# MarkTakken/kf2vecFSW

Hardware: AMD Instinct MI355X
Metric: Gbases/s k-mer→.kf build at k=7; achieved HBM GB/s vs gfx950 peak (higher is better)
Workload: dtype u32

## Files before the change

kf2vecfsw_amd/build.py:

```python
from __future__ import annotations

import hashlib
import os
import subprocess
import sys

HERE = os.path.dirname(os.path.abspath(__file__))
CSRC = os.path.join(HERE, "csrc")
OUT = os.path.join(HERE, "libkf2vec_gpu.so")
BUILD = os.path.join(HERE, "_build")
ARCH = os.environ.get("KF_OFFLOAD_ARCH", "gfx950")
HIPCC = os.environ.get("HIPCC", "/opt/rocm/bin/hipcc")

SOURCES_HIP = ["kf_count.hip", "kf_bucket.hip", "kf_chunks.hip", "kf_sparse.hip", "kf_index.hip", "kf_rows.hip",
               "kf_kmers.hip", "kf_merge.hip", "kf_chunkfeat.hip", "kf_kfparse.hip"]
SOURCES_CPP = ["kf_host.cpp"]
DEPS = SOURCES_HIP + SOURCES_CPP + ["kf_internal.h", "kf_front.h", "kf_scan.h", "kf_compact.h", "../../include/kf2vec_gpu.h"]


def source_id() -> str:
    h = hashlib.sha256(ARCH.encode())
    for d in sorted(DEPS):
        h.update(b"\0" + os.path.basename(d).encode() + b"\0")
        with open(os.path.join(CSRC, d), "rb") as f:
            h.update(f.read())
    return h.hexdigest()[:16]


def embedded_id(path: str) -> str | None:
    try:
        with open(path, "rb") as f:
            blob = f.read()
    except OSError:
        return None
    i = blob.find(b"KF_BUILD_ID=")
    if i < 0:
        return None
    j = blob.find(b"\0", i)
    return blob[i + 12: j].decode(errors="replace")


def _stale() -> bool:
    return embedded_id(OUT) != source_id()


def build(force: bool = False, verbose: bool = False, ablation: bool = False, out: str | None = None) -> str:
    import fcntl
    out = out or OUT
    if not force and not ablation and out == OUT and not _stale():
        return OUT
    os.makedirs(BUILD, exist_ok=True)
    with open(os.path.join(BUILD, ".lock"), "w") as lk:
        fcntl.flock(lk, fcntl.LOCK_EX)
        if not force and not ablation and out == OUT and not _stale():
            return OUT
        return _build_locked(verbose, ablation, out)


HEADERS = ["kf_internal.h", "kf_front.h", "kf_scan.h", "kf_compact.h", "../../include/kf2vec_gpu.h"]

_TOOLCHAIN: list[bytes] = []


def _toolchain_id() -> bytes:
    if not _TOOLCHAIN:
        out = b""
        for cmd in ([HIPCC, "--version"], ["g++", "--version"]):
            try:
                out += subprocess.run(cmd, capture_output=True, check=False).stdout
            except OSError:
                out += b"missing:" + cmd[0].encode()
        _TOOLCHAIN.append(out)
    return _TOOLCHAIN[0]


def _object(src: str, cmd_tail: list[str], csrc: str = CSRC) -> tuple[str, bool]:
    h = hashlib.sha256(" ".join(cmd_tail).encode() + b"\0" + _toolchain_id())
    for d in [src] + HEADERS:
        with open(os.path.join(csrc, d), "rb") as f:
            h.update(f.read())
    o = os.path.join(BUILD, f"{src}.{h.hexdigest()[:16]}.o")
    return o, os.path.exists(o)


ABL_PATCHES = [os.path.join(HERE, "..", "tools", "zoo", "bucket_ablations.patch")]


def _ablation_sources() -> str:
    import shutil
    root = os.path.join(BUILD, "abl_src")
    shutil.rmtree(root, ignore_errors=True)
    shutil.copytree(CSRC, os.path.join(root, "kf2vecfsw_amd", "csrc"))
# ... 79 lines not shown
```

kf2vecfsw_amd/csrc/kf_bucket.hip:

```cpp
#include <hip/hip_runtime.h>
#include <stdint.h>
#include <stdlib.h>

#include <algorithm>
#include <cstdio>
#include <mutex>
#include <vector>

#include "kf_front.h"
#include "kf_internal.h"

namespace kf {


constexpr int kBkWaves = 16;
constexpr int kBkBits = 15;
constexpr uint64_t kPieceMax = (8ull << 20) - (64ull << 10);
constexpr uint32_t kBkLagShift = 3;
constexpr uint32_t kBkSlots = 2;
constexpr uint32_t kBkRoundWeights = 0x060B1114;
constexpr int kBkGroupWindows = 4;
constexpr bool bk_pre2(int K) { return K <= 10; }
constexpr uint32_t bk_rl(int K) { return K == 10 ? 4 : 0; }

// ... 858 lines not shown
        double sum[8] = {0, 0, 0, 0, 0, 0, 0, 0};
        for (int i = 0; i < grid; ++i)
            for (int x = 0; x < 8; ++x) sum[x] += (double)prof_h[8 * i + x];
        const double np = sum[2] > 0 ? sum[2] : 1;
        int occ = 0;
        (void)hipOccupancyMaxActiveBlocksPerMultiprocessor(&occ, (const void*)fn, waves * kWave, lds);
        fprintf(stderr, "[kf_bucket k=%d] grid %d x %d waves, LDS %u B, resident workgroups per CU %d\n", k, grid,
                waves, lds, occ);
        fprintf(stderr, "[kf_bucket k=%d] pieces %.0f cycles/piece: phase1 %.3g phase2 %.3g "
                "(records %.3g, barrier %.3g, flush %.3g, barrier %.3g)\n",
                k, sum[2], sum[0] / np, sum[1] / np, sum[3] / np, sum[4] / np, sum[5] / np, sum[6] / np);
        fprintf(stderr, "[kf_bucket k=%d] per wave, cycles per piece:", k);
        for (int w = 0; w < waves; ++w) {
            double v[4] = {0, 0, 0, 0};
            for (int i = 0; i < grid; ++i)
                for (int x = 0; x < 4; ++x) v[x] += (double)prof_h[8 * grid + 4 * (waves * i + w) + x];
            fprintf(stderr, "\n  w%d records %.3g (consume %.3g) barrier %.3g | phase-1 barrier %.3g", w, v[0] / np,
                    v[3] / np, v[1] / np, v[2] / np);
        }
        fprintf(stderr, "\n");
    }
    return KF_OK;
}

}

extern "C" int kf_workspace_release(void) {
    int dev = 0;
    if (hipGetDevice(&dev) != hipSuccess) return kf_fail(KF_EHIP, "hipGetDevice failed");
    if (dev < 0 || dev >= 64) return kf_fail(KF_EINVAL, "device index out of range");
    std::lock_guard<std::mutex> lk(g_mu);
    DevState& d = g_dev[dev];
    if (hipDeviceSynchronize() != hipSuccess) return kf_fail(KF_EHIP, "hipDeviceSynchronize failed");
    for (int k = 0; k <= KF_MAX_K; ++k) {
        if (d.col_idx[k]) (void)hipFree(d.col_idx[k]);
        if (d.bcol[k]) (void)hipFree(d.bcol[k]);
        d.col_idx[k] = nullptr;
        d.bcol[k] = nullptr;
    }
    if (d.scratch) (void)hipFree(d.scratch);
    if (d.pstart) (void)hipFree(d.pstart);
    d.scratch = nullptr;
    d.scratch_bytes = 0;
    d.pstart = nullptr;
    d.pstart_n = 0;
    return KF_OK;
}
```

kf2vecfsw_amd/csrc/kf_count.hip:

```cpp
#include <hip/hip_runtime.h>
#include <stdint.h>
#include <stdlib.h>

#include <mutex>

#include "kf_front.h"
#include "kf_internal.h"

namespace kf {

constexpr int kBlock = 1024;
constexpr uint32_t kWaveWeights = 20u | 17u << 8 | 11u << 16 | 6u << 24;
constexpr int kXRing = 2;

__device__ __forceinline__ void wg_span(const CountArgs& A, uint64_t& lo, uint64_t& hi) {
    const uint64_t base = A.goff[0];
    const uint64_t total = A.goff[A.n_genomes] - base;
    const uint64_t G = gridDim.x, b = blockIdx.x;
    lo = base + ((total / G * b + (total % G) * b / G) & ~(uint64_t)15);
    hi = (b + 1 == G) ? base + total : base + ((total / G * (b + 1) + (total % G) * (b + 1) / G) & ~(uint64_t)15);
}

template <int K>
struct XL {
    static constexpr uint32_t P = K >= 8 ? (1u << 17) : (2u << (2 * (K + 1)));
    static constexpr uint32_t S = K >= 8 ? (1u << 15) : (2u << (2 * K));
    static constexpr uint32_t bytes = P + S;
};
constexpr int kXChunk = 3 * kChunk;
static_assert((uint32_t)kXChunk == kLattice, "wave ranges are split on the iteration lattice (split_at_lattice)");
constexpr uint32_t kLatticeMaxIters = 2560;
constexpr uint32_t kHot7 = 0xC000C000u, kStep7 = 0x4000u;
constexpr uint32_t kHot8 = 0xE000E000u, kStep8 = 0x2000u;
constexpr uint32_t kHot6 = 0x80008000u, kStep6 = 0x8000u;
template <int K>
constexpr uint32_t x_hot() { return K >= 8 ? kHot8 : (K == 7 ? kHot7 : kHot6); }
template <int K>
constexpr uint32_t x_step() { return K >= 8 ? kStep8 : (K == 7 ? kStep7 : kStep6); }

__device__ __forceinline__ uint32_t k9_code_of(uint32_t i) { return ((i >> 9) << 10) | (i & 0x1FFu); }

__device__ __forceinline__ uint32_t half_one(uint32_t i) { return 1u << ((i & 1u) << 4); }

template <int B>
__device__ __forceinline__ uint32_t shl1_byte(uint32_t h, uint32_t one) {
    uint32_t r;
    if constexpr (B == 0)
        asm("v_lshlrev_b32_sdwa %0, %1, %2 dst_sel:DWORD dst_unused:UNUSED_PAD src0_sel:BYTE_0 src1_sel:DWORD"
            : "=v"(r) : "v"(h), "v"(one));
    else if constexpr (B == 1)
        asm("v_lshlrev_b32_sdwa %0, %1, %2 dst_sel:DWORD dst_unused:UNUSED_PAD src0_sel:BYTE_1 src1_sel:DWORD"
            : "=v"(r) : "v"(h), "v"(one));
    else if constexpr (B == 2)
        asm("v_lshlrev_b32_sdwa %0, %1, %2 dst_sel:DWORD dst_unused:UNUSED_PAD src0_sel:BYTE_2 src1_sel:DWORD"
            : "=v"(r) : "v"(h), "v"(one));
    else
        asm("v_lshlrev_b32_sdwa %0, %1, %2 dst_sel:DWORD dst_unused:UNUSED_PAD src0_sel:BYTE_3 src1_sel:DWORD"
            : "=v"(r) : "v"(h), "v"(one));
    return r;
}
// ... 282 lines not shown
}

template <int K, bool MASKED>
__device__ __forceinline__ uint32_t x_singles(const uint4 d, const CountArgs& A, uint64_t chunk, int lane,
                                              const ChunkMask& m, uint64_t iv0, uint32_t carry, uint32_t* gcounts,
                                              uint32_t& lane_total, uint32_t& drained) {
    constexpr uint32_t HOT = x_hot<K>();
    uint32_t C, V, EN, ne, own;
    front_end<K, MASKED, false>(d, A, chunk, lane, m, iv0, C, V, EN, ne, own);
    const Windows win = windows<K, MASKED>(C, V, EN, ne, carry, lane);
    const uint32_t wlo = win.wlo, whi = win.whi, R = win.R;
    if constexpr (K == 9) {
        drained |= k9b_region<false>(wlo, whi, R, A, gcounts);
        lane_total += (uint32_t)__builtin_popcount(R);
        return win.next;
    }
    const uint32_t wv[4] = {wlo, __builtin_amdgcn_alignbit(whi, wlo, 8), __builtin_amdgcn_alignbit(whi, wlo, 16),
                            __builtin_amdgcn_alignbit(whi, wlo, 24)};
    uint32_t o = 0;
#pragma unroll
    for (int r = 0; r < 16; ++r) {
        const int fo = (2 * r) & ~7;
        const uint32_t y = __builtin_amdgcn_ubfe(wv[fo >> 3], 2 * r - fo, 2 * K);
        o |= lds_add_rtn((K == 8 ? 0u : XL<K>::P) + ((y >> 1) << 2), ((R >> r) & 1u) * half_one(y));
    }
    if (__builtin_amdgcn_ballot_w64((o & HOT) != 0) != 0) {
        x_scan_drain<K>(A.code2col, gcounts, lane);
        drained = 1;
    }
    lane_total += (uint32_t)__builtin_popcount(R);
    return win.next;
}

template <int K>
__device__ __forceinline__ uint32_t x_range(const CountArgs& A, int32_t g, uint64_t glo, uint64_t ghi, uint64_t lo,
                                            uint64_t hi, int lane, uint64_t& iv_hint, uint32_t& drained) {
    if (lo >= hi) return 0;
    uint32_t* gcounts = A.counts + (uint64_t)g * A.nbins;
    Range rg;
    rg.init(glo, ghi, lo, hi);
    auto load = [&](uint32_t r) {
        return xc_load(A.bytes, rg.c0, r, rg.end_r, lane);
    };
    static_assert(kXRing == 2, "two-deep register ring");
    XBlock buf[K == 9 ? 1 : kXRing];
    XBlock b0, b1;
    if constexpr (K == 9) {
        b0 = load(0);
        b1 = load(kXChunk);
    } else {
#pragma unroll
        for (int j = 0; j < kXRing; ++j) buf[j] = load(j * kXChunk);
    }
    const uint32_t nx = (rg.nch + 2) / 3;
    rg.warm16<K>(A, lane, iv_hint);
    __builtin_amdgcn_s_setprio(0);
    uint32_t carry = rg.carry;
    uint32_t rel = 0;
    const ChunkMask m = rg.mask();
    uint32_t lane_total = 0;
    uint32_t nfast = 0;
    auto step = [&](const XBlock& bf) {
        bool fast = !rg.masked_span(A, rel, kXChunk);
        if (fast)
            fast = xc_fast<K>(bf, A, lane, carry, gcounts, lane_total, drained);
        nfast += fast ? 1u : 0u;
        if (!fast) {
            const bool m0 = rg.masked(A, rel);
            const uint64_t iv0 = rg.iv;
            const bool m1 = rg.masked(A, rel + kChunk);
            const uint64_t iv1 = rg.iv;
// ... 50 lines not shown
#pragma unroll
        for (int a = 0; a < 4; ++a) {
            const uint32_t v = hist[a * 8192 + i * 1024 + tid];
            F[2 * i] += v & 0xFFFFu;
            F[2 * i + 1] += v >> 16;
        }
    }
}

template <int K>
__device__ __forceinline__ void pair_f_sums_small(const uint32_t* hist, int tid,
                                                  uint32_t (&F)[((1u << (2 * K)) + kBlock - 1) / kBlock]) {
    constexpr uint32_t NY = 1u << (2 * K), NM = (NY + kBlock - 1) / kBlock;
#pragma unroll
    for (uint32_t m = 0; m < NM; ++m) {
        const uint32_t y = (uint32_t)tid + kBlock * m;
        F[m] = 0;
        if (y < NY) {
            const uint32_t sh = (y & 1u) << 4;
            uint32_t f = u16sum2(hist[2 * y]) + u16sum2(hist[2 * y + 1]);
#pragma unroll
            for (uint32_t a = 0; a < 4; ++a) f += (hist[a * (NY / 2) + (y >> 1)] >> sh) & 0xFFFFu;
            f += (hist[XL<K>::P / 4 + (y >> 1)] >> sh) & 0xFFFFu;
            F[m] = f;
        }
    }
}

__device__ __forceinline__ void lds_zero(uint32_t* hist, uint32_t lo4, uint32_t hi4, int tid) {
    uint4* h4 = (uint4*)hist;
    for (uint32_t i = lo4 + (uint32_t)tid; i < hi4; i += kBlock) h4[i] = make_uint4(0u, 0u, 0u, 0u);
}

template <int K>
__global__ void __launch_bounds__(kBlock) __attribute__((amdgpu_waves_per_eu(4, 4))) k1x_kernel(CountArgs A) {
    static_assert(K >= 2 && K <= 9, "K1x serves k = 2 .. 9 (k = 9: K9b byte counters)");
    extern __shared__ __attribute__((aligned(16))) uint32_t hist[];
    const int tid = threadIdx.x;
    const int lane = tid & (kWave - 1);
    const int wave = __builtin_amdgcn_readfirstlane(tid >> 6);
    {
        uint4* h4 = (uint4*)hist;
        for (uint32_t i = tid; i < XL<K>::bytes / 16; i += kBlock) h4[i] = make_uint4(0u, 0u, 0u, 0u);
    }
    __syncthreads();
    if ((uint32_t)(uintptr_t)(lds_u32*)hist != 0u) __builtin_trap();
    uint64_t span_lo, span_hi;
    wg_span(A, span_lo, span_hi);
    if (span_lo >= span_hi) return;
    int32_t g = (int32_t)wave_upper_bound((uint64_t)A.n_genomes, span_lo, lane,
                                          [&](uint64_t i) { return A.goff[i + 1]; });
    const uint32_t fr_lo = wave_frac((uint32_t)wave, kWaveWeights), fr_hi = wave_frac((uint32_t)wave + 1, kWaveWeights);
    uint64_t g_lo = A.goff[g], g_hi = A.goff[g + 1];
    uint64_t iv_hint = 0;
    for (; g < A.n_genomes; ++g) {
        __builtin_amdgcn_s_setprio(3);
        const uint64_t glo = g_lo, ghi = g_hi;
        g_lo = g_hi;
        g_hi = A.goff[min(g + 2, A.n_genomes)];
        if (glo >= span_hi) break;
        const uint64_t plo = max(glo, span_lo), phi = min(ghi, span_hi);
        if (phi <= plo) continue;
        const uint32_t nit = lattice_iters(plo, phi);
        const bool lat = nit <= kLatticeMaxIters;
        const uint64_t lo = split_at_lattice(plo, phi, nit, lat, fr_lo), hi = split_at_lattice(plo, phi, nit, lat, fr_hi);
        uint32_t drained = 0;
        unsigned long long s = x_range<K>(A, g, glo, ghi, lo, hi, lane, iv_hint, drained);
        uint32_t* gc = A.counts + (uint64_t)g * A.nbins;
        const bool whole = plo == glo && phi == ghi && !(A.flags & KF_ACCUMULATE);
        if constexpr (K == 9) {
            lds_barrier();
            if (lane == 0) hist[XL<K>::P / 4 + wave] = drained;
            lds_barrier();
            const uint4* fl = (const uint4*)(hist + XL<K>::P / 4);
            const uint4 f0 = fl[0], f1 = fl[1], f2 = fl[2], f3 = fl[3];
            const bool any_fix = (f0.x | f0.y | f0.z | f0.w | f1.x | f1.y | f1.z | f1.w | f2.x | f2.y | f2.z |
                                  f2.w | f3.x | f3.y | f3.z | f3.w) != 0;
            const uint8_t* hb = (const uint8_t*)hist;
            for (uint32_t c0 = (uint32_t)tid; c0 < (1u << 17); c0 += 4 * kBlock) {
                uint32_t rep[4];
#pragma unroll
                for (int j = 0; j < 4; ++j) rep[j] = A.col2rep[c0 + j * kBlock];
#pragma unroll
                for (int j = 0; j < 4; ++j) {
                    const uint32_t c = (rep[j] & 0x200u) ? kf_revcomp<9>(rep[j]) : rep[j];
                    const uint32_t v = hb[((c >> 1) & 0x1FE00u) | (c & 0x1FFu)];
                    if (whole && !any_fix)
                        __builtin_nontemporal_store(v, gc + c0 + j * kBlock);
                    else if (v)
                        __hip_atomic_fetch_add(gc + c0 + j * kBlock, v, __ATOMIC_RELAXED, __HIP_MEMORY_SCOPE_AGENT);
                }
            }
            lds_barrier();
            uint4* h4 = (uint4*)hist;
            for (uint32_t i = tid; i < XL<K>::bytes / 16; i += kBlock) h4[i] = make_uint4(0u, 0u, 0u, 0u);
        } else if constexpr (K == 8) {
            lds_barrier();
            if (lane == 0) hist[XL<K>::P / 4 + wave] = drained;
            lds_barrier();
            const uint4* fl = (const uint4*)(hist + XL<K>::P / 4);
            const uint4 f0 = fl[0], f1 = fl[1], f2 = fl[2], f3 = fl[3];
            const bool any_drain = (f0.x | f0.y | f0.z | f0.w | f1.x | f1.y | f1.z | f1.w | f2.x | f2.y | f2.z |
                                    f2.w | f3.x | f3.y | f3.z | f3.w) != 0;
            for (uint32_t col = tid; col < A.nbins; col += kBlock) {
                const uint32_t y = A.col2rep[col], rc = kf_revcomp<8>(y);
                uint32_t v = (hist[y >> 1] >> ((y & 1u) << 4)) & 0xFFFFu;
                if (rc != y) v += (hist[rc >> 1] >> ((rc & 1u) << 4)) & 0xFFFFu;
                if (whole && !any_drain)
                    gc[col] = v;
                else if (v)
                    __hip_atomic_fetch_add(gc + col, v, __ATOMIC_RELAXED, __HIP_MEMORY_SCOPE_AGENT);
            }
            lds_barrier();
            uint4* h4 = (uint4*)hist;
            for (uint32_t i = tid; i < XL<K>::bytes / 16; i += kBlock) h4[i] = make_uint4(0u, 0u, 0u, 0u);
        } else if constexpr (K <= 6) {
            constexpr uint32_t NY = 1u << (2 * K), NM = (NY + kBlock - 1) / kBlock;
            constexpr uint32_t NCOL = (NY + (K % 2 == 0 ? (1u << K) : 0u)) / 2, NC = (NCOL + kBlock - 1) / kBlock;
            constexpr uint32_t ZF = (NY + 16) / 4;
            static_assert(ZF <= XL<K>::bytes / 16, "F and the flags lie inside the table");
            uint32_t rep[NC];
#pragma unroll
            for (uint32_t c = 0; c < NC; ++c) {
                const uint32_t col = (uint32_t)tid + c * kBlock;
                rep[c] = col < NCOL ? A.col2rep[col] : 0u;
            }
            lds_barrier();
            uint32_t F[NM];
            pair_f_sums_small<K>(hist, tid, F);
            lds_barrier();
#pragma unroll
            for (uint32_t m = 0; m < NM; ++m) {
                const uint32_t y = (uint32_t)tid + kBlock * m;
                if (y < NY) hist[f_swz(y)] = F[m];
            }
            if (lane == 0) hist[NY + wave] = drained;
            lds_zero(hist, ZF, XL<K>::bytes / 16, tid);
            lds_barrier();
            const uint4* fl = (const uint4*)(hist + NY);
            const uint4 f0 = fl[0], f1 = fl[1], f2 = fl[2], f3 = fl[3];
            const bool any_drain = (f0.x | f0.y | f0.z | f0.w | f1.x | f1.y | f1.z | f1.w | f2.x | f2.y | f2.z | f2.w |
                                    f3.x | f3.y | f3.z | f3.w) != 0;
            uint32_t cv[NC];
#pragma unroll
            for (uint32_t c = 0; c < NC; ++c) {
                const uint32_t y = rep[c], rc = kf_revcomp<K>(y);
                cv[c] = hist[f_swz(y)] + (rc != y ? hist[f_swz(rc)] : 0u);
            }
            lds_barrier();
            lds_zero(hist, 0, ZF, tid);
#pragma unroll
            for (uint32_t c = 0; c < NC; ++c) {
                const uint32_t col = (uint32_t)tid + c * kBlock;
                if (col >= NCOL) continue;
                if (whole && !any_drain)
                    __builtin_nontemporal_store(cv[c], gc + col);
                else if (cv[c])
                    __hip_atomic_fetch_add(gc + col, cv[c], __ATOMIC_RELAXED, __HIP_MEMORY_SCOPE_AGENT);
            }
        } else {
            uint32_t rep[8];
            if (whole) {
                const uint4 r0 = *(const uint4*)(A.col2rep + 4 * tid), r1 = *(const uint4*)(A.col2rep + 4096 + 4 * tid);
                rep[0] = r0.x, rep[1] = r0.y, rep[2] = r0.z, rep[3] = r0.w;
                rep[4] = r1.x, rep[5] = r1.y, rep[6] = r1.z, rep[7] = r1.w;
            } else {
#pragma unroll
                for (int c = 0; c < 8; ++c) rep[c] = A.col2rep[tid + c * kBlock];
            }
            lds_barrier();
            uint32_t F[16];
            pair_f_sums(hist, tid, F);
#pragma unroll
            for (int i = 0; i < 8; ++i) {
                const uint32_t v = hist[XL<K>::P / 4 + i * 1024 + tid];
                F[2 * i] += v & 0xFFFFu;
                F[2 * i + 1] += v >> 16;
            }
            lds_barrier();
#pragma unroll
            for (int i = 0; i < 8; ++i) *(uint2*)(hist + f_swz(i * 2048 + 2 * tid)) = make_uint2(F[2 * i], F[2 * i + 1]);
            if (lane == 0) hist[16384 + wave] = drained;
            constexpr uint32_t ZF = (16384 + 16) / 4;
            lds_zero(hist, ZF, XL<K>::bytes / 16, tid);
            lds_barrier();
            const uint4* fl = (const uint4*)(hist + 16384);
            const uint4 f0 = fl[0], f1 = fl[1], f2 = fl[2], f3 = fl[3];
            const bool any_drain = (f0.x | f0.y | f0.z | f0.w | f1.x | f1.y | f1.z | f1.w | f2.x | f2.y | f2.z | f2.w |
                                    f3.x | f3.y | f3.z | f3.w) != 0;
            uint32_t cv[8];
#pragma unroll
            for (int c = 0; c < 8; ++c) {
                const uint32_t y = rep[c], rc = kf_revcomp<7>(y);
                cv[c] = hist[f_swz(y)] + hist[f_swz(rc)];
            }
            lds_barrier();
            lds_zero(hist, 0, ZF, tid);
            if (whole && !any_drain) {
                typedef unsigned int v4u_t __attribute__((ext_vector_type(4)));
                __builtin_nontemporal_store(v4u_t{cv[0], cv[1], cv[2], cv[3]}, (v4u_t*)(gc + 4 * tid));
                __builtin_nontemporal_store(v4u_t{cv[4], cv[5], cv[6], cv[7]}, (v4u_t*)(gc + 4096 + 4 * tid));
            } else {
#pragma unroll
                for (int c = 0; c < 8; ++c) {
                    const uint32_t col = whole ? (c >> 2) * 4096 + 4 * tid + (c & 3) : tid + c * kBlock;
                    if (cv[c]) __hip_atomic_fetch_add(gc + col, cv[c], __ATOMIC_RELAXED, __HIP_MEMORY_SCOPE_AGENT);
                }
            }
        }
        s = wave_sum(s);
        if (lane == 0 && s) atomicAdd(A.totals + g, s);
        lds_barrier();
    }
}

__device__ __forceinline__ uint64_t splitmix64(uint64_t x) {
    x += 0x9E3779B97F4A7C15ull;
    x = (x ^ (x >> 30)) * 0xBF58476D1CE4E5B9ull;
    x = (x ^ (x >> 27)) * 0x94D049BB133111EBull;
    return x ^ (x >> 31);
}

__device__ __forceinline__ bool in_nrun(uint64_t key, uint64_t i, uint64_t n_period) {
    if (!n_period) return false;
    uint64_t b = i >> 12;
    for (int d = 0; d < 2; ++d) {
        if (d == 1) {
            if (b == 0) break;
            b -= 1;
        }
        const uint64_t h = splitmix64((key ^ 0xA5A5A5A5A5A5A5A5ull) + b);
        if (h % n_period) continue;
        const uint64_t st = (b << 12) + ((h >> 16) % 4096), ln = 1 + ((h >> 32) % 100);
        if (i >= st && i < st + ln) return true;
    }
    return false;
}

__global__ void __launch_bounds__(256) synth_kernel(uint8_t* bytes, const uint64_t* goff, int64_t g0, int64_t gstride,
                                                     uint64_t seed0, uint64_t seq_len, int width, uint64_t n_period) {
    const int32_t gi = blockIdx.y;
    const uint64_t lo = goff[gi], hi = goff[gi + 1];
    const int64_t g = g0 + gi * gstride;
    char digits[24];
// ... 50 lines not shown
    const uint64_t w = (uint64_t)blockIdx.x * (blockDim.x / kWave) + (threadIdx.x >> 6);
    constexpr uint32_t kB = 3 * kChunk;
    const uint64_t nblk = (n + kB - 1) / kB;
    uint32_t acc = 0;
    for (uint64_t b = w; b < nblk; b += 4 * nw) {
        uint4 v[4][3];
#pragma unroll
        for (int k = 0; k < 4; ++k) {
            const uint64_t bb = b + (uint64_t)k * nw;
            const uint64_t base = bb < nblk ? bb * kB : 0;
            const int rec = bb < nblk ? (int)min((uint64_t)kB, n - base) : 0;
            const auto rs = __builtin_amdgcn_make_buffer_rsrc((void*)(bytes + base), (short)0, rec, 0x00020000);
#pragma unroll
            for (int q = 0; q < 3; ++q) {
                const auto t = __builtin_amdgcn_raw_buffer_load_b128(rs, 16 * lane + 1024 * q, 0, 0);
                v[k][q] = make_uint4(t[0], t[1], t[2], t[3]);
            }
        }
#pragma unroll
        for (int k = 0; k < 4; ++k)
#pragma unroll
            for (int q = 0; q < 3; ++q) acc ^= v[k][q].x ^ v[k][q].y ^ v[k][q].z ^ v[k][q].w;
    }
    acc = wave_xor(acc);
    if (lane == 0 && acc) atomicXor(out, acc);
}

}

using namespace kf;

namespace {

void* kernel_for(int k) {
    switch (k) {
    case 2: return (void*)&k1x_kernel<2>;
    case 3: return (void*)&k1x_kernel<3>;
    case 4: return (void*)&k1x_kernel<4>;
    case 5: return (void*)&k1x_kernel<5>;
    case 6: return (void*)&k1x_kernel<6>;
    case 7: return (void*)&k1x_kernel<7>;
    case 8: return (void*)&k1x_kernel<8>;
    case 9: return (void*)&k1x_kernel<9>;
    default: return nullptr;
    }
}

int lds_bytes_for(int k) {
    switch (k) {
    case 2: return (int)XL<2>::bytes;
    case 3: return (int)XL<3>::bytes;
    case 4: return (int)XL<4>::bytes;
    case 5: return (int)XL<5>::bytes;
    case 6: return (int)XL<6>::bytes;
    case 7: return (int)XL<7>::bytes;
    case 8: return (int)XL<8>::bytes;
    default: return (int)XL<9>::bytes;
    }
}


int g_grid[KF_MAX_K + 1][64];
std::mutex g_grid_mu;

int launch_info(int k, int* grid, int* block, int* lds) {
    int dev = 0;
    if (hipGetDevice(&dev) != hipSuccess) return kf_fail(KF_EHIP, "hipGetDevice failed");
    if (dev < 0 || dev >= 64) return kf_fail(KF_EINVAL, "device index out of range");
    const int l = lds_bytes_for(k);
    std::lock_guard<std::mutex> lk(g_grid_mu);
    int& gr = g_grid[k][dev];
    if (!gr) {
        void* fn = kernel_for(k);
        if (hipFuncSetAttribute(fn, hipFuncAttributeMaxDynamicSharedMemorySize, l) != hipSuccess)
            return kf_fail(KF_EHIP, "hipFuncSetAttribute(MaxDynamicSharedMemorySize) failed");
        int per_cu = 0, cus = 0;
        if (hipOccupancyMaxActiveBlocksPerMultiprocessor(&per_cu, fn, kBlock, l) != hipSuccess)
            return kf_fail(KF_EHIP, "hipOccupancyMaxActiveBlocksPerMultiprocessor failed");
        if (hipDeviceGetAttribute(&cus, hipDeviceAttributeMultiprocessorCount, dev) != hipSuccess)
            return kf_fail(KF_EHIP, "hipDeviceGetAttribute(MultiprocessorCount) failed");
        gr = (per_cu < 1 ? 1 : per_cu) * (cus > 0 ? cus : 1);
    }
    *grid = gr;
    *block = kBlock;
    *lds = l;
    return KF_OK;
}
}

extern "C" int kf_count_launch_info(int k, int* grid, int* block, int* lds_bytes) {
    if (k < KF_MIN_K || k > KF_MAX_K) return kf_fail(KF_EINVAL, "k out of range [2, 12]");
    if (!grid || !block || !lds_bytes) return kf_fail(KF_EINVAL, "null output pointer");
    if (k >= 10) return bucket_launch_info(k, grid, block, lds_bytes);
    return launch_info(k, grid, block, lds_bytes);
}

extern "C" int kf_workspace_reserve(int k, int32_t max_genomes) {
    if (k < KF_MIN_K || k > KF_MAX_K) return kf_fail(KF_EINVAL, "k out of range [2, 12]");
    if (max_genomes < 0) return kf_fail(KF_EINVAL, "max_genomes < 0");
    if (k >= 10) return bucket_reserve(k, max_genomes);
    int grid = 0, block = 0, lds = 0;
    return launch_info(k, &grid, &block, &lds);
}

extern "C" int kf_count_batch(const uint8_t* d_bytes, const uint64_t* d_goff, int32_t n_genomes,
                              const uint64_t* d_excl, uint64_t n_excl, const uint32_t* d_code2col,
                              const uint32_t* d_col2rep, int k, uint32_t* d_counts, uint64_t* d_totals,
                              uint32_t flags, void* stream) {
    if (k < KF_MIN_K || k > KF_MAX_K) return kf_fail(KF_EINVAL, "k out of range [2, 12]");
    if (n_genomes < 0) return kf_fail(KF_EINVAL, "n_genomes < 0");
    if (n_genomes == 0) return KF_OK;
    if (!d_bytes || !d_goff || !d_counts || !d_totals || !d_code2col || !d_col2rep)
        return kf_fail(KF_EINVAL, "null device pointer");
    if (n_excl && !d_excl) return kf_fail(KF_EINVAL, "d_excl is null but n_excl > 0");
    if (((uintptr_t)d_bytes) & 15) return kf_fail(KF_EINVAL, "d_bytes must be 16-byte aligned");
    const uint64_t nb = kf_num_bins(k);
    hipStream_t s = (hipStream_t)stream;
    const bool bucket = k >= 10;
    if (!(flags & KF_ACCUMULATE)) {
        if ((!bucket && hipMemsetAsync(d_counts, 0, (size_t)n_genomes * nb * sizeof(uint32_t), s) != hipSuccess) ||
            hipMemsetAsync(d_totals, 0, (size_t)n_genomes * sizeof(uint64_t), s) != hipSuccess)
            return kf_fail(KF_EHIP, "hipMemsetAsync failed");
    }
    CountArgs A;
    A.bytes = d_bytes;
    A.goff = d_goff;
    A.excl = d_excl;
    A.n_excl = n_excl;
    A.code2col = d_code2col;
    A.col2rep = d_col2rep;
    A.counts = d_counts;
    A.totals = (unsigned long long*)d_totals;
    A.nbins = (uint32_t)nb;
    A.n_genomes = n_genomes;
    A.flags = flags;
    if (bucket) return bucket_launch(A, k, flags, s);
    int grid = 0, block = 0, lds = 0;
    const int rc = launch_info(k, &grid, &block, &lds);
    if (rc) return rc;

    void* args[] = {&A};
    if (hipLaunchKernel(kernel_for(k), dim3(grid), dim3(block), args, (size_t)lds, s) != hipSuccess)
        return kf_fail(KF_EHIP, "count kernel launch failed: %s", hipGetErrorString(hipGetLastError()));
    return KF_OK;
}

extern "C" int kf_stream_probe(const uint8_t* d_bytes, uint64_t n, uint32_t* d_out, void* stream) {
    if (!d_bytes || !d_out) return kf_fail(KF_EINVAL, "null device pointer");
    if (((uintptr_t)d_bytes) & 15) return kf_fail(KF_EINVAL, "d_bytes must be 16-byte aligned");
    if (n == 0) return KF_OK;
    int dev = 0, cus = 0;
    if (hipGetDevice(&dev) != hipSuccess ||
        hipDeviceGetAttribute(&cus, hipDeviceAttributeMultiprocessorCount, dev) != hipSuccess)
        return kf_fail(KF_EHIP, "device query failed");
    hipLaunchKernelGGL(stream_probe_kernel, dim3(2 * (cus > 0 ? cus : 1)), dim3(1024), 0, (hipStream_t)stream, d_bytes,
                       n, d_out);
    if (hipGetLastError() != hipSuccess) return kf_fail(KF_EHIP, "stream probe launch failed");
    return KF_OK;
}

extern "C" int kf_synth_fasta(uint8_t* d_bytes, const uint64_t* d_goff, int32_t n_genomes, int64_t g0,
                              int64_t g_stride, uint64_t seed0, uint64_t seq_len, int width, uint64_t n_period,
                              void* stream) {
    if (n_genomes <= 0) return n_genomes == 0 ? KF_OK : kf_fail(KF_EINVAL, "n_genomes < 0");
    if (!d_bytes || !d_goff) return kf_fail(KF_EINVAL, "null device pointer");
    if (width < 1) return kf_fail(KF_EINVAL, "width < 1");
    if (n_genomes > 65535) return kf_fail(KF_EINVAL, "at most 65535 genomes per synth call");
    dim3 grid(512, (unsigned)n_genomes);
    hipLaunchKernelGGL(synth_kernel, grid, dim3(256), 0, (hipStream_t)stream, d_bytes, d_goff, g0, g_stride, seed0,
                       seq_len, width, n_period);
    if (hipGetLastError() != hipSuccess) return kf_fail(KF_EHIP, "synth kernel launch failed");
    return KF_OK;
}
```

kf2vecfsw_amd/csrc/kf_front.h:

```cpp
#pragma once
#include <hip/hip_runtime.h>
#include <stdint.h>

#include "kf_scan.h"

namespace kf {

constexpr int kWave = 64;
constexpr int kChunk = 1024;

struct CountArgs {
    const uint8_t* bytes;
    const uint64_t* goff;
    const uint64_t* excl;
    uint64_t n_excl;
    const uint32_t* code2col;
    const uint32_t* col2rep;
    uint32_t* counts;
    unsigned long long* totals;
    uint32_t nbins;
    int32_t n_genomes;
    uint32_t flags;
};

__device__ __forceinline__ uint32_t tail_pack(uint32_t codes, uint32_t n, uint32_t ne) {
    return codes | (min(n, 31u) << 22) | (min(ne, 31u) << 27);
}
__device__ __forceinline__ uint32_t t_codes(uint32_t t) { return t & 0x3FFFFFu; }
__device__ __forceinline__ uint32_t t_n(uint32_t t) { return (t >> 22) & 31u; }
__device__ __forceinline__ uint32_t t_ne(uint32_t t) { return t >> 27; }

template <int K>
__device__ __forceinline__ uint32_t tail_combine(uint32_t a, uint32_t b) {
    constexpr uint32_t TM = (K > 1) ? ((1u << (2 * (K - 1))) - 1u) : 0u;
    const uint32_t bn = t_n(b), bne = t_ne(b);
    const uint32_t n = (bn < bne) ? bn : min(t_n(a) + bn, 31u);
    const uint32_t codes =
        (bne >= (uint32_t)(K - 1)) ? t_codes(b) : (((t_codes(a) << (2 * bne)) | t_codes(b)) & TM);
    return tail_pack(codes, n, t_ne(a) + bne);
}
template <int K>
__device__ __forceinline__ bool tail_complete(uint32_t t) {
    return t_n(t) < t_ne(t) || t_n(t) >= (uint32_t)(K - 1);
}

__device__ __forceinline__ void classify16(const uint4 d, uint32_t& C, uint32_t& INV, uint32_t& NNL) {
    const uint32_t w[4] = {d.x, d.y, d.z, d.w};
    uint32_t pc[4], vf[4], nf[4];
#pragma unroll
    for (int q = 0; q < 4; ++q) {
        const uint32_t x = w[q];
        const uint32_t cb = (x >> 1) & 0x03030303u;
        const uint32_t ex = __builtin_amdgcn_perm(0u, 0x4B584F4Du, cb);
        const uint32_t y = (x ^ ex) & 0xDFDFDFDFu;
        vf[q] = __builtin_amdgcn_perm(0xFFFFFFFFu, 0xFFFFFFFFu, y);
// ... 378 lines not shown
};
template <int K, bool MASKED>
__device__ __forceinline__ Windows windows(uint32_t C, uint32_t V, uint32_t EN, uint32_t ne, uint32_t carry,
                                           int lane) {
    constexpr uint32_t TM = (K > 1) ? ((1u << (2 * (K - 1))) - 1u) : 0u;
    const uint32_t own = own_tail<K>(C, V, ne);
    uint32_t ctx = wave_shr1(carry, own);
    if (__ballot(ne < (uint32_t)(K - 1)) != 0) {
        const uint64_t inc_mask = __ballot(!tail_complete<K>(own)) & 0x7FFFFFFFFFFFFFFFull;
        if (inc_mask) ctx = scan_ctx<K>(own, carry, lane);
    }
    const uint64_t W = ((uint64_t)t_codes(ctx) << (2 * ne)) | (uint64_t)C;
    Windows w;
    w.wlo = (uint32_t)W;
    w.whi = (uint32_t)(W >> 32);
    const uint32_t ctxlen = min(t_n(ctx), (uint32_t)(K - 1));
    const uint32_t E = (((1u << ctxlen) - 1u) << ne) | V;
    w.R = run_mask<K>(E) & ((1u << ne) - 1u);
    if (MASKED) w.R &= EN;
    const uint32_t incl = tail_pack(w.wlo & TM, (uint32_t)__builtin_ctz(~E), 31u);
    w.next = (uint32_t)__builtin_amdgcn_readlane((int)incl, kWave - 1);
    return w;
}

__device__ __forceinline__ unsigned long long wave_sum(unsigned long long v) {
#pragma unroll
    for (int d = 32; d >= 1; d >>= 1) v += __shfl_xor(v, d, kWave);
    return v;
}

int bucket_launch(const CountArgs& A, int k, uint32_t flags, hipStream_t s);
int bucket_launch_info(int k, int* grid, int* block, int* lds);
int bucket_reserve(int k, int32_t max_genomes);

}
```

Baseline: 5856.

## Replace k<=7 memsets and global atomics with per-block partial rows plus merge kernel

New measurement: 5625. 0.96x the previous value.

```diff
diff --git a/kf2vecfsw_amd/build.py b/kf2vecfsw_amd/build.py
--- a/kf2vecfsw_amd/build.py
+++ b/kf2vecfsw_amd/build.py
@@ -15,7 +15,8 @@
 SOURCES_HIP = ["kf_count.hip", "kf_bucket.hip", "kf_chunks.hip", "kf_sparse.hip", "kf_index.hip", "kf_rows.hip",
                "kf_kmers.hip", "kf_merge.hip", "kf_chunkfeat.hip", "kf_kfparse.hip"]
 SOURCES_CPP = ["kf_host.cpp"]
-DEPS = SOURCES_HIP + SOURCES_CPP + ["kf_internal.h", "kf_front.h", "kf_scan.h", "kf_compact.h", "../../include/kf2vec_gpu.h"]
+DEPS = SOURCES_HIP + SOURCES_CPP + ["kf_internal.h", "kf_front.h", "kf_scan.h", "kf_compact.h", "kf_span.h",
+                                    "../../include/kf2vec_gpu.h"]
 
 
 def source_id() -> str:
@@ -57,7 +58,7 @@
         return _build_locked(verbose, ablation, out)
 
 
-HEADERS = ["kf_internal.h", "kf_front.h", "kf_scan.h", "kf_compact.h", "../../include/kf2vec_gpu.h"]
+HEADERS = ["kf_internal.h", "kf_front.h", "kf_scan.h", "kf_compact.h", "kf_span.h", "../../include/kf2vec_gpu.h"]
 
 _TOOLCHAIN: list[bytes] = []
 
diff --git a/kf2vecfsw_amd/csrc/kf_bucket.hip b/kf2vecfsw_amd/csrc/kf_bucket.hip
--- a/kf2vecfsw_amd/csrc/kf_bucket.hip
+++ b/kf2vecfsw_amd/csrc/kf_bucket.hip
@@ -914,6 +914,7 @@
     std::lock_guard<std::mutex> lk(g_mu);
     DevState& d = g_dev[dev];
     if (hipDeviceSynchronize() != hipSuccess) return kf_fail(KF_EHIP, "hipDeviceSynchronize failed");
+    count_ws_release(dev);
     for (int k = 0; k <= KF_MAX_K; ++k) {
         if (d.col_idx[k]) (void)hipFree(d.col_idx[k]);
         if (d.bcol[k]) (void)hipFree(d.bcol[k]);
diff --git a/kf2vecfsw_amd/csrc/kf_count.hip b/kf2vecfsw_amd/csrc/kf_count.hip
--- a/kf2vecfsw_amd/csrc/kf_count.hip
+++ b/kf2vecfsw_amd/csrc/kf_count.hip
@@ -2,10 +2,12 @@
 #include <stdint.h>
 #include <stdlib.h>
 
+#include <algorithm>
 #include <mutex>
 
 #include "kf_front.h"
 #include "kf_internal.h"
+#include "kf_span.h"
 
 namespace kf {
 
@@ -15,17 +17,130 @@
 
 __device__ __forceinline__ void wg_span(const CountArgs& A, uint64_t& lo, uint64_t& hi) {
     const uint64_t base = A.goff[0];
-    const uint64_t total = A.goff[A.n_genomes] - base;
-    const uint64_t G = gridDim.x, b = blockIdx.x;
-    lo = base + ((total / G * b + (total % G) * b / G) & ~(uint64_t)15);
-    hi = (b + 1 == G) ? base + total : base + ((total / G * (b + 1) + (total % G) * (b + 1) / G) & ~(uint64_t)15);
+    wg_span(A.goff[A.n_genomes] - base, gridDim.x, blockIdx.x, lo, hi);
+    lo += base;
+    hi += base;
+}
+
+constexpr uint32_t kWsRow = 8192;
+static_assert(KF_MAX_K >= 7, "the workspace rows are sized for k = 7");
+template <int K>
+constexpr uint32_t x_ncol() { return ((1u << (2 * K)) + (K % 2 == 0 ? (1u << K) : 0u)) / 2; }
+template <int K>
+struct XCols {
+    static constexpr int N = K == 7 ? 8 : (int)((x_ncol<K>() + 1023) / 1024);
+    uint32_t v[N];
+};
+template <int K, class F>
+__device__ __forceinline__ void cols_each4(int tid, F f) {
+    static_assert(K == 7, "16-byte accesses: k = 7");
+    f(4u * (uint32_t)tid, 0);
+    f(4096u + 4u * (uint32_t)tid, 4);
+}
+template <int K>
+__device__ __forceinline__ void cols_store(uint32_t* row, const XCols<K>& c, int tid) {
+    if constexpr (K == 7) {
+        cols_each4<K>(tid, [&](uint32_t col, int i) {
+            *(uint4*)(row + col) = make_uint4(c.v[i], c.v[i + 1], c.v[i + 2], c.v[i + 3]);
+        });
+    } else {
+#pragma unroll
+        for (int i = 0; i < XCols<K>::N; ++i) {
+            const uint32_t col = (uint32_t)tid + 1024u * i;
+            if (col < x_ncol<K>()) row[col] = c.v[i];
+        }
+    }
+}
+template <int K>
+__device__ __forceinline__ void cols_add(const uint32_t* row, XCols<K>& c, int tid) {
+    if constexpr (K == 7) {
+        cols_each4<K>(tid, [&](uint32_t col, int i) {
+            const uint4 w = *(const uint4*)(row + col);
+            c.v[i] += w.x, c.v[i + 1] += w.y, c.v[i + 2] += w.z, c.v[i + 3] += w.w;
+        });
+    } else {
+#pragma unroll
+        for (int i = 0; i < XCols<K>::N; ++i) {
+            const uint32_t col = (uint32_t)tid + 1024u * i;
+            if (col < x_ncol<K>()) c.v[i] += row[col];
+        }
+    }
+}
+template <int K>
+__device__ __forceinline__ void cols_take_drain(uint32_t* drain, XCols<K>& c, int tid) {
+#pragma unroll
+    for (int i = 0; i < XCols<K>::N; ++i) {
+        const uint32_t col = K == 7 ? (uint32_t)(i >> 2) * 4096u + 4u * (uint32_t)tid + (uint32_t)(i & 3)
+                                    : (uint32_t)tid + 1024u * i;
+        if (K == 7 || col < x_ncol<K>())
+            c.v[i] += __hip_atomic_exchange(drain + col, 0u, __ATOMIC_RELAXED, __HIP_MEMORY_SCOPE_AGENT);
+    }
+}
+
+__device__ __noinline__ void x_zero_row(uint32_t* gc, uint32_t nbins, unsigned long long* total, int tid) {
+    for (uint32_t c = (uint32_t)tid; c < nbins; c += kBlock) gc[c] = 0u;
+    if (tid == 0) *total = 0ull;
+}
+
+struct PartArgs {
+    uint32_t* gc;
+    unsigned long long* total;
+    uint32_t* ws_rows;
+    unsigned long long* ws_tot;
+};
+constexpr uint32_t kPartDrain = 1u, kPartWhole = 2u, kPartHead = 4u;
+
+template <int K>
+__device__ __noinline__ void x_part(PartArgs P, uint32_t kind, XCols<K> c, unsigned long long tot) {
+    const int tid = threadIdx.x;
+    const uint64_t b = blockIdx.x;
+    if (kind & kPartDrain) cols_take_drain<K>(P.ws_rows + (3 * b + 2) * kWsRow, c, tid);
+    if (kind & kPartWhole) {
+        cols_store<K>(P.gc, c, tid);
+        if (tid == 0) *P.total = tot;
+        return;
+    }
+    const uint64_t mine = 2 * b + ((kind & kPartHead) ? 0u : 1u);
+    cols_store<K>(P.ws_rows + (mine + b) * kWsRow, c, tid);
+    if (tid == 0) P.ws_tot[mine] = tot;
+}
+
+template <int K>
+__global__ void __launch_bounds__(kBlock) x_merge_kernel(CountArgs A) {
+    const int tid = threadIdx.x;
+    const uint64_t b = blockIdx.x, G = gridDim.x;
+    const uint64_t base = A.goff[0], total = A.goff[A.n_genomes] - base;
+    uint64_t lo, hi;
+    wg_span(total, G, b, lo, hi);
+    if (lo >= hi) return;
+    lo += base, hi += base;
+    const int32_t g = (int32_t)wave_upper_bound((uint64_t)A.n_genomes, hi - 1, tid & (kWave - 1),
+                                                [&](uint64_t i) { return A.goff[i + 1]; });
+    const uint64_t glo = A.goff[g], ghi = A.goff[g + 1];
+    if (glo < lo || ghi <= hi) return;
+    XCols<K> c;
+#pragma unroll
+    for (int i = 0; i < XCols<K>::N; ++i) c.v[i] = 0u;
+    cols_add<K>(A.ws_rows + (3 * b + 1) * kWsRow, c, tid);
+    unsigned long long tot = A.ws_tot[2 * b + 1];
+    for (uint64_t w = b + 1; w < G; ++w) {
+        uint64_t slo, shi;
+        wg_span(total, G, w, slo, shi);
+        if (slo + base >= ghi) break;
+        if (shi <= slo) continue;
+        cols_add<K>(A.ws_rows + 3 * w * kWsRow, c, tid);
+        tot += A.ws_tot[2 * w];
+    }
+    cols_store<K>(A.counts + (uint64_t)g * A.nbins, c, tid);
+    if (tid == 0) A.totals[g] = tot;
 }
 
 template <int K>
 struct XL {
     static constexpr uint32_t P = K >= 8 ? (1u << 17) : (2u << (2 * (K + 1)));
     static constexpr uint32_t S = K >= 8 ? (1u << 15) : (2u << (2 * K));
-    static constexpr uint32_t bytes = P + S;
+    static constexpr uint32_t flush = K <= 7 ? 4u * ((1u << (2 * K)) + 48u) : 0u;
+    static constexpr uint32_t bytes = P + S > flush ? P + S : flush;
 };
 constexpr int kXChunk = 3 * kChunk;
 static_assert((uint32_t)kXChunk == kLattice, "wave ranges are split on the iteration lattice (split_at_lattice)");
@@ -374,11 +489,11 @@
     return win.next;
 }
 
-template <int K>
+template <int K, bool ONE>
 __device__ __forceinline__ uint32_t x_range(const CountArgs& A, int32_t g, uint64_t glo, uint64_t ghi, uint64_t lo,
                                             uint64_t hi, int lane, uint64_t& iv_hint, uint32_t& drained) {
     if (lo >= hi) return 0;
-    uint32_t* gcounts = A.counts + (uint64_t)g * A.nbins;
+    uint32_t* gcounts = ONE ? A.ws_rows + (3 * (uint64_t)blockIdx.x + 2) * kWsRow : A.counts + (uint64_t)g * A.nbins;
     Range rg;
     rg.init(glo, ghi, lo, hi);
     auto load = [&](uint32_t r) {
@@ -495,9 +610,10 @@
     for (uint32_t i = lo4 + (uint32_t)tid; i < hi4; i += kBlock) h4[i] = make_uint4(0u, 0u, 0u, 0u);
 }
 
-template <int K>
+template <int K, bool ONE = false>
 __global__ void __launch_bounds__(kBlock) __attribute__((amdgpu_waves_per_eu(4, 4))) k1x_kernel(CountArgs A) {
     static_assert(K >= 2 && K <= 9, "K1x serves k = 2 .. 9 (k = 9: K9b byte counters)");
+    static_assert(!ONE || K <= 7, "no memsets: k <= 7");
     extern __shared__ __attribute__((aligned(16))) uint32_t hist[];
     const int tid = threadIdx.x;
     const int lane = tid & (kWave - 1);
@@ -510,9 +626,12 @@
     if ((uint32_t)(uintptr_t)(lds_u32*)hist != 0u) __builtin_trap();
     uint64_t span_lo, span_hi;
     wg_span(A, span_lo, span_hi);
-    if (span_lo >= span_hi) return;
-    int32_t g = (int32_t)wave_upper_bound((uint64_t)A.n_genomes, span_lo, lane,
-                                          [&](uint64_t i) { return A.goff[i + 1]; });
+    const bool owns_end = ONE && blockIdx.x + 1 == gridDim.x;
+    if (span_lo >= span_hi && !owns_end) return;
+    int32_t g = ONE && span_lo == A.goff[0]
+                    ? 0
+                    : (int32_t)wave_upper_bound((uint64_t)A.n_genomes, span_lo - (ONE ? 1u : 0u), lane,
+                                                [&](uint64_t i) { return A.goff[i + 1]; });
     const uint32_t fr_lo = wave_frac((uint32_t)wave, kWaveWeights), fr_hi = wave_frac((uint32_t)wave + 1, kWaveWeights);
     uint64_t g_lo = A.goff[g], g_hi = A.goff[g + 1];
     uint64_t iv_hint = 0;
@@ -521,16 +640,39 @@
         const uint64_t glo = g_lo, ghi = g_hi;
         g_lo = g_hi;
         g_hi = A.goff[min(g + 2, A.n_genomes)];
-        if (glo >= span_hi) break;
+        if (glo >= span_hi && !owns_end) break;
         const uint64_t plo = max(glo, span_lo), phi = min(ghi, span_hi);
-        if (phi <= plo) continue;
+        if (phi <= plo) {
+            if (ONE && glo == ghi) x_zero_row(A.counts + (uint64_t)g * A.nbins, A.nbins, A.totals + g, tid);
+            continue;
+        }
         const uint32_t nit = lattice_iters(plo, phi);
         const bool lat = nit <= kLatticeMaxIters;
         const uint64_t lo = split_at_lattice(plo, phi, nit, lat, fr_lo), hi = split_at_lattice(plo, phi, nit, lat, fr_hi);
         uint32_t drained = 0;
-        unsigned long long s = x_range<K>(A, g, glo, ghi, lo, hi, lane, iv_hint, drained);
+        unsigned long long s = x_range<K, ONE>(A, g, glo, ghi, lo, hi, lane, iv_hint, drained);
         uint32_t* gc = A.counts + (uint64_t)g * A.nbins;
-        const bool whole = plo == glo && phi == ghi && !(A.flags & KF_ACCUMULATE);
+        const bool whole = plo == glo && phi == ghi && (ONE || !(A.flags & KF_ACCUMULATE));
+        unsigned long long tot = 0;
+        if constexpr (ONE) {
+            s = wave_sum(s);
+            if (drained) asm volatile("s_waitcnt vmcnt(0)" ::: "memory");
+        }
+        auto part = [&](const auto& cols, bool any_drain) {
+            if constexpr (ONE) {
+                PartArgs P;
+                P.gc = gc, P.total = A.totals + g, P.ws_rows = A.ws_rows, P.ws_tot = A.ws_tot;
+                x_part<K>(P, (any_drain ? kPartDrain : 0u) | (whole ? kPartWhole : 0u) | (glo < span_lo ? kPartHead : 0u),
+                          cols, tot);
+            }
+        };
+        auto wave_totals = [&](uint32_t w0) {
+            if (wave == 0) {
+                unsigned long long v = 0;
+                if (lane < 16) v = *(const unsigned long long*)(hist + w0 + 2 * lane);
+                tot = wave_sum(v);
+            }
+        };
         if constexpr (K == 9) {
             lds_barrier();
             if (lane == 0) hist[XL<K>::P / 4 + wave] = drained;
@@ -580,8 +722,8 @@
         } else if constexpr (K <= 6) {
             constexpr uint32_t NY = 1u << (2 * K), NM = (NY + kBlock - 1) / kBlock;
             constexpr uint32_t NCOL = (NY + (K % 2 == 0 ? (1u << K) : 0u)) / 2, NC = (NCOL + kBlock - 1) / kBlock;
-            constexpr uint32_t ZF = (NY + 16) / 4;
-            static_assert(ZF <= XL<K>::bytes / 16, "F and the flags lie inside the table");
+            constexpr uint32_t ZF = (NY + 16 + (ONE ? 32 : 0)) / 4;
+            static_assert(ZF <= XL<K>::bytes / 16, "F, the flags and the totals lie inside the table");
             uint32_t rep[NC];
 #pragma unroll
             for (uint32_t c = 0; c < NC; ++c) {
@@ -598,6 +740,7 @@
                 if (y < NY) hist[f_swz(y)] = F[m];
             }
             if (lane == 0) hist[NY + wave] = drained;
+            if (ONE && lane == 0) *(unsigned long long*)(hist + NY + 16 + 2 * wave) = s;
             lds_zero(hist, ZF, XL<K>::bytes / 16, tid);
             lds_barrier();
             const uint4* fl = (const uint4*)(hist + NY);
@@ -610,20 +753,38 @@
                 const uint32_t y = rep[c], rc = kf_revcomp<K>(y);
                 cv[c] = hist[f_swz(y)] + (rc != y ? hist[f_swz(rc)] : 0u);
             }
+            if constexpr (ONE) wave_totals(NY + 16);
             lds_barrier();
             lds_zero(hist, 0, ZF, tid);
-#pragma unroll
-            for (uint32_t c = 0; c < NC; ++c) {
-                const uint32_t col = (uint32_t)tid + c * kBlock;
-                if (col >= NCOL) continue;
-                if (whole && !any_drain)
-                    __builtin_nontemporal_store(cv[c], gc + col);
-                else if (cv[c])
-                    __hip_atomic_fetch_add(gc + col, cv[c], __ATOMIC_RELAXED, __HIP_MEMORY_SCOPE_AGENT);
+            if constexpr (ONE) {
+                if (whole && !any_drain) {
+#pragma unroll
+                    for (uint32_t c = 0; c < NC; ++c) {
+                        const uint32_t col = (uint32_t)tid + c * kBlock;
+                        if (col < NCOL) __builtin_nontemporal_store(cv[c], gc + col);
+                    }
+                    if (tid == 0) A.totals[g] = tot;
+                } else {
+                    XCols<K> cols;
+                    static_assert(XCols<K>::N == (int)NC && x_ncol<K>() == NCOL, "x_part's columns are the flush's");
+#pragma unroll
+                    for (uint32_t c = 0; c < NC; ++c) cols.v[c] = cv[c];
+                    part(cols, any_drain);
+                }
+            } else {
+#pragma unroll
+                for (uint32_t c = 0; c < NC; ++c) {
+                    const uint32_t col = (uint32_t)tid + c * kBlock;
+                    if (col >= NCOL) continue;
+                    if (whole && !any_drain)
+                        __builtin_nontemporal_store(cv[c], gc + col);
+                    else if (cv[c])
+                        __hip_atomic_fetch_add(gc + col, cv[c], __ATOMIC_RELAXED, __HIP_MEMORY_SCOPE_AGENT);
+                }
             }
         } else {
             uint32_t rep[8];
-            if (whole) {
+            if (ONE || whole) {
                 const uint4 r0 = *(const uint4*)(A.col2rep + 4 * tid), r1 = *(const uint4*)(A.col2rep + 4096 + 4 * tid);
                 rep[0] = r0.x, rep[1] = r0.y, rep[2] = r0.z, rep[3] = r0.w;
                 rep[4] = r1.x, rep[5] = r1.y, rep[6] = r1.z, rep[7] = r1.w;
@@ -644,7 +805,8 @@
 #pragma unroll
             for (int i = 0; i < 8; ++i) *(uint2*)(hist + f_swz(i * 2048 + 2 * tid)) = make_uint2(F[2 * i], F[2 * i + 1]);
             if (lane == 0) hist[16384 + wave] = drained;
-            constexpr uint32_t ZF = (16384 + 16) / 4;
+            if (ONE && lane == 0) *(unsigned long long*)(hist + 16400 + 2 * wave) = s;
+            constexpr uint32_t ZF = (16384 + 16 + (ONE ? 32 : 0)) / 4;
             lds_zero(hist, ZF, XL<K>::bytes / 16, tid);
             lds_barrier();
             const uint4* fl = (const uint4*)(hist + 16384);
@@ -657,12 +819,19 @@
                 const uint32_t y = rep[c], rc = kf_revcomp<7>(y);
                 cv[c] = hist[f_swz(y)] + hist[f_swz(rc)];
             }
+            if constexpr (ONE) wave_totals(16400);
             lds_barrier();
             lds_zero(hist, 0, ZF, tid);
             if (whole && !any_drain) {
                 typedef unsigned int v4u_t __attribute__((ext_vector_type(4)));
                 __builtin_nontemporal_store(v4u_t{cv[0], cv[1], cv[2], cv[3]}, (v4u_t*)(gc + 4 * tid));
                 __builtin_nontemporal_store(v4u_t{cv[4], cv[5], cv[6], cv[7]}, (v4u_t*)(gc + 4096 + 4 * tid));
+                if (ONE && tid == 0) A.totals[g] = tot;
+            } else if constexpr (ONE) {
+                XCols<K> cols;
+#pragma unroll
+                for (int c = 0; c < 8; ++c) cols.v[c] = cv[c];
+                part(cols, any_drain);
             } else {
 #pragma unroll
                 for (int c = 0; c < 8; ++c) {
@@ -671,8 +840,10 @@
                 }
             }
         }
-        s = wave_sum(s);
-        if (lane == 0 && s) atomicAdd(A.totals + g, s);
+        if constexpr (!ONE) {
+            s = wave_sum(s);
+            if (lane == 0 && s) atomicAdd(A.totals + g, s);
+        }
         lds_barrier();
     }
 }
@@ -789,7 +960,20 @@
 
 namespace {
 
-void* kernel_for(int k) {
+bool one_launch(int k, uint32_t flags) { return k <= 7 && !(flags & KF_ACCUMULATE); }
+
+void* kernel_for(int k, bool one = false) {
+    if (one) {
+        switch (k) {
+        case 2: return (void*)&k1x_kernel<2, true>;
+        case 3: return (void*)&k1x_kernel<3, true>;
+        case 4: return (void*)&k1x_kernel<4, true>;
+        case 5: return (void*)&k1x_kernel<5, true>;
+        case 6: return (void*)&k1x_kernel<6, true>;
+        case 7: return (void*)&k1x_kernel<7, true>;
+        default: return nullptr;
+        }
+    }
     switch (k) {
     case 2: return (void*)&k1x_kernel<2>;
     case 3: return (void*)&k1x_kernel<3>;
@@ -803,6 +987,18 @@
     }
 }
 
+void* merge_kernel_for(int k) {
+    switch (k) {
+    case 2: return (void*)&x_merge_kernel<2>;
+    case 3: return (void*)&x_merge_kernel<3>;
+    case 4: return (void*)&x_merge_kernel<4>;
+    case 5: return (void*)&x_merge_kernel<5>;
+    case 6: return (void*)&x_merge_kernel<6>;
+    case 7: return (void*)&x_merge_kernel<7>;
+    default: return nullptr;
+    }
+}
+
 int lds_bytes_for(int k) {
     switch (k) {
     case 2: return (int)XL<2>::bytes;
@@ -829,7 +1025,9 @@
     int& gr = g_grid[k][dev];
     if (!gr) {
         void* fn = kernel_for(k);
-        if (hipFuncSetAttribute(fn, hipFuncAttributeMaxDynamicSharedMemorySize, l) != hipSuccess)
+        if (hipFuncSetAttribute(fn, hipFuncAttributeMaxDynamicSharedMemorySize, l) != hipSuccess ||
+            (one_launch(k, 0) &&
+             hipFuncSetAttribute(kernel_for(k, true), hipFuncAttributeMaxDynamicSharedMemorySize, l) != hipSuccess))
             return kf_fail(KF_EHIP, "hipFuncSetAttribute(MaxDynamicSharedMemorySize) failed");
         int per_cu = 0, cus = 0;
         if (hipOccupancyMaxActiveBlocksPerMultiprocessor(&per_cu, fn, kBlock, l) != hipSuccess)
@@ -843,6 +1041,47 @@
     *lds = l;
     return KF_OK;
 }
+
+struct OneWs {
+    uint32_t* rows = nullptr;
+    unsigned long long* tot = nullptr;
+    int grid = 0;
+    hipEvent_t done = nullptr;
+    hipStream_t last = nullptr;
+    bool used = false;
+};
+OneWs g_one[64];
+std::mutex g_one_mu;
+
+int ensure_one(OneWs& w, int grid) {
+    if (!w.done && hipEventCreateWithFlags(&w.done, hipEventDisableTiming) != hipSuccess)
+        return kf_fail(KF_EHIP, "hipEventCreate failed");
+    if (w.grid < grid) {
+        if (w.rows && (hipDeviceSynchronize() != hipSuccess || hipFree(w.rows) != hipSuccess))
+            return kf_fail(KF_EHIP, "hipFree of the k <= 7 workspace failed");
+        w.rows = nullptr;
+        w.grid = 0;
+        const size_t rows_b = (size_t)grid * 3 * kWsRow * sizeof(uint32_t), tot_b = (size_t)grid * 2 * 8;
+        if (hipMalloc((void**)&w.rows, rows_b + tot_b) != hipSuccess)
+            return kf_fail(KF_EHIP, "hipMalloc of %zu bytes of k <= 7 workspace failed", rows_b + tot_b);
+        if (hipMemset(w.rows, 0, rows_b + tot_b) != hipSuccess || hipDeviceSynchronize() != hipSuccess)
+            return kf_fail(KF_EHIP, "zeroing the k <= 7 workspace failed");
+        w.tot = (unsigned long long*)((char*)w.rows + rows_b);
+        w.grid = grid;
+    }
+    return KF_OK;
+}
+}
+
+namespace kf {
+void count_ws_release(int dev) {
+    std::lock_guard<std::mutex> lk(g_one_mu);
+    OneWs& w = g_one[dev];
+    if (w.rows) (void)hipFree(w.rows);
+    w.rows = nullptr, w.tot = nullptr;
+    w.grid = 0;
+    w.used = false, w.last = nullptr;
+}
 }
 
 extern "C" int kf_count_launch_info(int k, int* grid, int* block, int* lds_bytes) {
@@ -857,7 +1096,12 @@
     if (max_genomes < 0) return kf_fail(KF_EINVAL, "max_genomes < 0");
     if (k >= 10) return bucket_reserve(k, max_genomes);
     int grid = 0, block = 0, lds = 0;
-    return launch_info(k, &grid, &block, &lds);
+    const int rc = launch_info(k, &grid, &block, &lds);
+    if (rc || !one_launch(k, 0)) return rc;
+    int dev = 0;
+    if (hipGetDevice(&dev) != hipSuccess) return kf_fail(KF_EHIP, "hipGetDevice failed");
+    std::lock_guard<std::mutex> lk(g_one_mu);
+    return ensure_one(g_one[dev], grid);
 }
 
 extern "C" int kf_count_batch(const uint8_t* d_bytes, const uint64_t* d_goff, int32_t n_genomes,
@@ -874,7 +1118,8 @@
     const uint64_t nb = kf_num_bins(k);
     hipStream_t s = (hipStream_t)stream;
     const bool bucket = k >= 10;
-    if (!(flags & KF_ACCUMULATE)) {
+    const bool one = one_launch(k, flags);
+    if (!(flags & KF_ACCUMULATE) && !one) {
         if ((!bucket && hipMemsetAsync(d_counts, 0, (size_t)n_genomes * nb * sizeof(uint32_t), s) != hipSuccess) ||
             hipMemsetAsync(d_totals, 0, (size_t)n_genomes * sizeof(uint64_t), s) != hipSuccess)
             return kf_fail(KF_EHIP, "hipMemsetAsync failed");
@@ -897,8 +1142,40 @@
     if (rc) return rc;
 
     void* args[] = {&A};
-    if (hipLaunchKernel(kernel_for(k), dim3(grid), dim3(block), args, (size_t)lds, s) != hipSuccess)
+    if (!one) {
+        if (hipLaunchKernel(kernel_for(k), dim3(grid), dim3(block), args, (size_t)lds, s) != hipSuccess)
+            return kf_fail(KF_EHIP, "count kernel launch failed: %s", hipGetErrorString(hipGetLastError()));
+        return KF_OK;
+    }
+    int dev = 0;
+    if (hipGetDevice(&dev) != hipSuccess) return kf_fail(KF_EHIP, "hipGetDevice failed");
+    std::lock_guard<std::mutex> lk(g_one_mu);
+    OneWs& w = g_one[dev];
+    const int rc1 = ensure_one(w, grid);
+    if (rc1) return rc1;
+    A.ws_rows = w.rows;
+    A.ws_tot = w.tot;
+    hipStreamCaptureStatus cap = hipStreamCaptureStatusNone;
+    if (hipStreamIsCapturing(s, &cap) != hipSuccess) return kf_fail(KF_EHIP, "hipStreamIsCapturing failed");
+    const bool live = cap == hipStreamCaptureStatusNone;
+    if (live && w.used && w.last != s) {
+        hipStreamCaptureStatus pc = hipStreamCaptureStatusNone;
+        const bool prev_ok = hipStreamIsCapturing(w.last, &pc) == hipSuccess && pc == hipStreamCaptureStatusNone &&
+                             hipEventRecord(w.done, w.last) == hipSuccess;
+        if (prev_ok) {
+            if (hipStreamWaitEvent(s, w.done, 0) != hipSuccess) return kf_fail(KF_EHIP, "hipStreamWaitEvent failed");
+        } else {
+            (void)hipGetLastError();
+            if (hipDeviceSynchronize() != hipSuccess) return kf_fail(KF_EHIP, "hipDeviceSynchronize failed");
+        }
+    }
+    if (hipLaunchKernel(kernel_for(k, true), dim3(grid), dim3(block), args, (size_t)lds, s) != hipSuccess ||
+        hipLaunchKernel(merge_kernel_for(k), dim3(grid), dim3(block), args, 0, s) != hipSuccess)
         return kf_fail(KF_EHIP, "count kernel launch failed: %s", hipGetErrorString(hipGetLastError()));
+    if (live) {
+        w.last = s;
+        w.used = true;
+    }
     return KF_OK;
 }
 
diff --git a/kf2vecfsw_amd/csrc/kf_front.h b/kf2vecfsw_amd/csrc/kf_front.h
--- a/kf2vecfsw_amd/csrc/kf_front.h
+++ b/kf2vecfsw_amd/csrc/kf_front.h
@@ -21,6 +21,8 @@
     uint32_t nbins;
     int32_t n_genomes;
     uint32_t flags;
+    uint32_t* ws_rows = nullptr;
+    unsigned long long* ws_tot = nullptr;
 };
 
 __device__ __forceinline__ uint32_t tail_pack(uint32_t codes, uint32_t n, uint32_t ne) {
@@ -465,5 +467,6 @@
 int bucket_launch(const CountArgs& A, int k, uint32_t flags, hipStream_t s);
 int bucket_launch_info(int k, int* grid, int* block, int* lds);
 int bucket_reserve(int k, int32_t max_genomes);
-
-}
+void count_ws_release(int dev);
+
+}
diff --git a/kf2vecfsw_amd/csrc/kf_span.h b/kf2vecfsw_amd/csrc/kf_span.h
--- /dev/null
+++ b/kf2vecfsw_amd/csrc/kf_span.h
@@ -0,0 +1,25 @@
+#pragma once
+#include <stdint.h>
+
+namespace kf {
+
+constexpr uint64_t span_cut(uint64_t total, uint64_t G, uint64_t b) {
+    return b >= G ? total : (total / G * b + (total % G) * b / G) & ~(uint64_t)15;
+}
+
+constexpr void wg_span(uint64_t total, uint64_t G, uint64_t b, uint64_t& lo, uint64_t& hi) {
+    lo = span_cut(total, G, b);
+    hi = span_cut(total, G, b + 1);
+}
+
+constexpr uint64_t wg_of(uint64_t total, uint64_t G, uint64_t off) {
+    uint64_t lo = 0, hi = G - 1;
+    while (lo < hi) {
+        const uint64_t mid = lo + (hi - lo + 1) / 2;
+        if (span_cut(total, G, mid) <= off) lo = mid;
+        else hi = mid - 1;
+    }
+    return lo;
+}
+
+}
```
